# AcherStyx/SSD-Object-Detection

Hardware: AMD Instinct MI355X
Metric: images/sec SSD300 train step, batch 64 (higher is better)
Workload: dtype bf16; 1 GPU; BASELINE configs[2]: SSD300 full train step (anchor match+encode, image normalisation, conv fwd, loss, conv bwd, per-variable clip (64 variables) + Adam), per-GPU batch 64, 80 classes, synthetic COCO-shaped boxes; per_gpu_batch=64, global_batch=64, parallelism=single

## Files before the change

### ssd-object-detection_amd/csrc/conv.hip

```cpp
#include <atomic>
#include <climits>
#include <cstdint>
#include <cstring>
#include <type_traits>
#include "common.h"
#include <hip/hip_bf16.h>
#include <stdlib.h>

namespace {

}
#include "conv_common.h"
namespace {

template <int EPI>
__global__ void k_igemm_finalize(ConvGeom g, Epilogue ep) {
    const int n4 = (g.N + 3) >> 2;
    const long long idx = (long long)blockIdx.x * blockDim.x + threadIdx.x;
    if (idx >= (long long)g.M * n4) return;
    const int m = (int)(idx / n4), n = (int)(idx - (long long)m * n4) * 4;
    const bool full = n + 3 < g.N;
    float v[4] = {0.f, 0.f, 0.f, 0.f};
    if (full && !(g.N & 3)) {
        for (int z = 0; z < ep.ksplit; ++z) {
// ... 395 lines not shown
        for (int c = 0; c < 2; ++c) { fw1[c][0] = ldf(cb + OFF_W1 + wf0 + c * 2048); fw1[c][1] = ldf(cb + OFF_W1 + wf1 + c * 2048); }
        if constexpr (!(ABL & 1)) issue_w(cb + OFF_W0, 0);
        SSD_PHASE_MMA(0, 1, fw1)
#pragma unroll
        for (int p = 0; p < 4; ++p) { fx[p][0] = ldf(cb + OFF_X1 + xf0 + p * 2048); fx[p][1] = ldf(cb + OFF_X1 + xf1 + p * 2048); }
        if constexpr (!(ABL & 1)) issue_x(cb + OFF_X0, 0);
        SSD_PHASE_MMA(1, 1, fw1)
        if constexpr (!(ABL & 1)) issue_w(cb + OFF_W1, 1);
        wq += 8;
        asm volatile("s_waitcnt vmcnt(6)" ::: "memory");
        SSD_PHASE_MMA(1, 0, fw0)
    }
#undef SSD_PHASE_MMA
    if (wr == 0) __builtin_amdgcn_s_barrier();

    if (staged_ok<EPI>(g, ep) && !(g.ablate & 8)) {
        asm volatile("s_waitcnt vmcnt(0)" ::: "memory");
        auto row_to_m = [&](int row) { const int m = m0 + row; return m < g.M ? m : -1; };
        staged_epilogue<EPI, 256, 256, 4, 8, 512>(acc, smem, g, ep, n0, wr * 128, wc * 64, tid, row_to_m);
        return;
    }
    int mrow[8];
#pragma unroll
    for (int p = 0; p < 8; ++p) {
        const int m = m0 + wr * 128 + p * 16 + (lane & 15);
        mrow[p] = m < g.M ? m : -1;
    }
    conv_epilogue_rows<EPI, 4, 8>(acc, g, ep, mrow, n0 + wc * 64, lane);
}

constexpr int PATCH_W = 18;
constexpr int PATCH_PIX = PATCH_W * PATCH_W;

__device__ __forceinline__ bf16x8_t lds_read_b128_scoped(const char* __restrict__ p, const char* __restrict__ other) {
    (void)other;
    return *reinterpret_cast<const bf16x8_t*>(p);
}
constexpr int P32_PITCH = 96;
constexpr int P32_PATCH = 32 * 1024;

template <int BN, int EPI, bool FLAT>
__global__ __launch_bounds__(512) __attribute__((amdgpu_waves_per_eu(4, 4))) void k_conv3x3_patch32(
    const bf16_raw* __restrict__ x, const bf16_raw* __restrict__ w, ConvGeom g, Epilogue ep, int tiles_x, int tiles_y, int nblocks, int rowflat) {
    constexpr int CT = BN / 32;
    constexpr int PT = 4;
    constexpr int WBYTES = BN * 64;
    constexpr int OFF_W = 2 * P32_PATCH;
    constexpr int OFF_DUMMY = OFF_W + 2 * WBYTES;
    extern __shared__ __attribute__((aligned(16))) char smem[];

    const int tid = threadIdx.x, lane = tid & 63;
    const int wave = __builtin_amdgcn_readfirstlane(tid >> 6);
    const int wave_m = wave & 3, wave_n = wave >> 2;
    const int ntn = (g.N + BN - 1) / BN;
    const int kx = blockIdx.x >> 3;
    const int pblock = (kx / ntn) * 8 + (blockIdx.x & 7);
    if (pblock >= nblocks) return;
    const int n0 = (kx % ntn) * BN;
    constexpr bool flat = FLAT;
    const int Q = FLAT ? g.W + 2 : PATCH_W;
    const int img = (g.H + 1) * Q;
    int b = 0, y0 = 0, x0 = 0, f0 = 0;
    if constexpr (FLAT) {
        f0 = pblock * 256;
    } else {
        int t = pblock;
        const int tx = t % tiles_x; t /= tiles_x;
        x0 = tx * 16;
        if (rowflat) { y0 = t * 16; }
        else { const int ty = t % tiles_y; b = t / tiles_y; y0 = ty * 16; }
    }
    auto image_row = [&](int r) {
        if (!rowflat) { const int y = y0 + r; return (unsigned)y < (unsigned)g.H ? b * g.H + y : -1; }
        const int R = y0 + r;
        if (R < 0) return -1;
        const int bb = fdiv(R, g.d_h1), yy = R - bb * (g.H + 1);
        return (bb < g.B && yy < g.H) ? bb * g.H + yy : -1;
    };
    auto flat_pixel = [&](int f) {
        if (f < 0) return -1;
        const int bb = f / img;
        const int r = f - bb * img;
        const int yy = r / Q, xx = r - yy * Q - 1;
        return (bb < g.B && yy < g.H && (unsigned)xx < (unsigned)g.W) ? (bb * g.H + yy) * g.W + xx : -1;
    };

    const __amdgpu_buffer_rsrc_t xres = __builtin_amdgcn_make_buffer_rsrc((void*)x, 0, (unsigned)g.B * g.H * g.W * g.C * 2u, 0x00020000);
    const __amdgpu_buffer_rsrc_t wres = __builtin_amdgcn_make_buffer_rsrc((void*)w, 0, (unsigned)g.N * (unsigned)g.ldw * 2u, 0x00020000);
    constexpr unsigned OOB = 0xfffffff0u;
    unsigned pvo[4];
#pragma unroll
    for (int j = 0; j < 4; ++j) {
        const int q = (wave + 8 * j) * 64 + lane;
        const int pp = q / 6, sl = q - pp * 6;
        int pix;
        if (flat) {
            pix = pp < 256 + 2 * (Q + 1) ? flat_pixel(f0 - (Q + 1) + pp) : -1;
        } else {
            const int py = pp / PATCH_W, px = pp - py * PATCH_W;
            const int ix = x0 - 1 + px;
            const int ir = pp < PATCH_PIX ? image_row(py - 1) : -1;
            pix = (ir >= 0 && (unsigned)ix < (unsigned)g.W) ? ir * g.W + ix : -1;
        }
        pvo[j] = (sl < 4 && pix >= 0) ? ((unsigned)pix * (unsigned)g.C + (unsigned)(sl * 8)) * 2u : OOB;
    }
    unsigned wvo;
    {
        const int row = 16 * wave + (lane >> 2);
        const int piece = (lane & 3) ^ ((-(row >> 2)) & 3);
        const int n = n0 + (BN == 64 ? (row & 63) : row);
        wvo = (row < (BN == 64 ? 128 : BN) && n < g.N) ? ((unsigned)n * (unsigned)g.ldw + (unsigned)(piece * 8)) * 2u : OOB;
    }
    const int wdst = wave < BN / 16 ? wave * 1024 : -1;
    const int nchunk = g.C >> 5;

    unsigned pstash[3];
    pstash[0] = pvo[1]; pstash[1] = pvo[2]; pstash[2] = pvo[3];
    asm volatile("" ::"v"(&pstash[0]) : "memory");
    const unsigned pvo0 = pvo[0];
    auto dma_patch = [&](int chunk, int buf) {
        const unsigned o1 = pstash[0], o2 = pstash[1], o3 = pstash[2];
        char* dst = smem + buf * P32_PATCH + wave * 1024;
        __builtin_amdgcn_raw_ptr_buffer_load_lds(xres, (lds_void*)dst, 16, pvo0, chunk * 64, 0, 0);
        __builtin_amdgcn_raw_ptr_buffer_load_lds(xres, (lds_void*)(dst + 8 * 1024), 16, o1, chunk * 64, 0, 0);
        __builtin_amdgcn_raw_ptr_buffer_load_lds(xres, (lds_void*)(dst + 16 * 1024), 16, o2, chunk * 64, 0, 0);
        __builtin_amdgcn_raw_ptr_buffer_load_lds(xres, (lds_void*)(dst + 24 * 1024), 16, o3, chunk * 64, 0, 0);
    };
    auto dma_w = [&](int chunk, int tap, int buf) {
        char* dst = wdst >= 0 ? smem + OFF_W + buf * WBYTES + wdst : smem + OFF_DUMMY;
        __builtin_amdgcn_raw_ptr_buffer_load_lds(wres, (lds_void*)dst, 16, wvo, (tap * g.C + chunk * 32) * 2, 0, 0);
    };

    f32x4_t acc[CT][PT];
#pragma unroll
    for (int c = 0; c < CT; ++c)
#pragma unroll
        for (int p = 0; p < PT; ++p) acc[c][p] = f32x4_t{0.f, 0.f, 0.f, 0.f};

    const int frow = lane & 15, fk = lane >> 4;
    const int xbase = (flat ? 4 * wave_m * 16 + frow : 4 * wave_m * PATCH_W + frow) * P32_PITCH + fk * 16;
    constexpr int prow = (FLAT ? 16 : PATCH_W) * P32_PITCH;
    int wbase;
    {
        const int row = wave_n * (16 * CT) + frow;
        wbase = OFF_W + row * 64 + ((fk ^ ((-(row >> 2)) & 3)) << 4);
    }
    auto ldf = [&](int addr) { return *reinterpret_cast<const bf16x8_t*>(smem + addr); };

    if constexpr (BN == 64) {
        constexpr int WB2 = 2 * WBYTES;
        auto dma_w2 = [&](int chunk, int step, int buf) {
            const int tap = 2 * step + (wave >> 2);
            __builtin_amdgcn_raw_ptr_buffer_load_lds(wres, (lds_void*)(smem + OFF_W + buf * WB2 + wave * 1024), 16,
                                                     tap <= 8 ? wvo : OOB, ((tap <= 8 ? tap : 8) * g.C + chunk * 32) * 2, 0, 0);
        };
        dma_patch(0, 0);
        dma_w2(0, 0, 0);
        for (int chunk = 0; chunk < nchunk; ++chunk) {
            const int pb = (chunk & 1) * P32_PATCH;
            const bool next_chunk = chunk + 1 < nchunk;
#pragma unroll
            for (int st = 0; st < 5; ++st) {
                const int sidx = chunk * 5 + st;
                const int wb = (sidx & 1) * WB2;
                if (st == 1 && next_chunk) asm volatile("s_waitcnt vmcnt(4) lgkmcnt(0)" ::: "memory");
                else asm volatile("s_waitcnt vmcnt(0) lgkmcnt(0)" ::: "memory");
                __builtin_amdgcn_s_barrier();
                if (!(g.ablate & 16)) {
                    if (st < 4) dma_w2(chunk, st + 1, (sidx + 1) & 1);
                    else if (next_chunk) dma_w2(chunk + 1, 0, (sidx + 1) & 1);
                }
                if (st == 0 && next_chunk && !(g.ablate & 32)) dma_patch(chunk + 1, (chunk + 1) & 1);
                bf16x8_t fx[2][PT], fw[2][CT];
#pragma unroll
                for (int t = 0; t < 2; ++t) {
                    const int tap = 2 * st + t;
                    if (tap > 8) continue;
                    const int tapoff = pb + xbase + ((tap / 3) * Q + tap % 3) * P32_PITCH;
#pragma unroll
                    for (int p = 0; p < PT; ++p) fx[t][p] = ldf(tapoff + p * prow);
#pragma unroll
                    for (int c = 0; c < CT; ++c) fw[t][c] = ldf(wb + wbase + t * WBYTES + c * 1024);
                }
                __builtin_amdgcn_s_setprio(0);
#pragma unroll
                for (int t = 0; t < 2; ++t) {
                    if (2 * st + t > 8) continue;
#pragma unroll
                    for (int c = 0; c < CT; ++c)
#pragma unroll
                        for (int p = 0; p < PT; ++p)
                            acc[c][p] = __builtin_amdgcn_mfma_f32_16x16x32_bf16(fw[t][c], fx[t][p], acc[c][p], 0, 0, 0);
                }
                __builtin_amdgcn_s_setprio(3);
            }
        }
    } else {
    dma_patch(0, 0);
    dma_w(0, 0, 0);
    for (int chunk = 0; chunk < nchunk; ++chunk) {
        const int pb = (chunk & 1) * P32_PATCH;
        const bool next_chunk = chunk + 1 < nchunk;
#pragma unroll
        for (int tap = 0; tap < 9; ++tap) {
            const int wb = ((chunk + tap) & 1) * WBYTES;
            if (tap == 1 && next_chunk) asm volatile("s_waitcnt vmcnt(4) lgkmcnt(0)" ::: "memory");
            else asm volatile("s_waitcnt vmcnt(0) lgkmcnt(0)" ::: "memory");
            __builtin_amdgcn_s_barrier();
            if (!(g.ablate & 16)) {
                if (tap < 8) dma_w(chunk, tap + 1, ((chunk + tap + 1) & 1));
                else if (next_chunk) dma_w(chunk + 1, 0, ((chunk + tap + 1) & 1));
            }
            if (tap == 0 && next_chunk && !(g.ablate & 32)) dma_patch(chunk + 1, (chunk + 1) & 1);
            bf16x8_t fx[PT], fw[CT];
            const int tapoff = pb + xbase + ((tap / 3) * Q + tap % 3) * P32_PITCH;
#pragma unroll
            for (int p = 0; p < PT; ++p) fx[p] = ldf(tapoff + p * prow);
#pragma unroll
            for (int c = 0; c < CT; ++c) fw[c] = ldf(wb + wbase + c * 1024);
            __builtin_amdgcn_s_setprio(0);
#pragma unroll
            for (int c = 0; c < CT; ++c)
#pragma unroll
                for (int p = 0; p < PT; ++p)
                    acc[c][p] = __builtin_amdgcn_mfma_f32_16x16x32_bf16(fw[c], fx[p], acc[c][p], 0, 0, 0);
            __builtin_amdgcn_s_setprio(3);
        }
    }
    }
    if (staged_ok<EPI>(g, ep) && !(g.ablate & 8)) {
        auto row_to_m = [&](int row) {
            if (flat) return flat_pixel(f0 + row);
            const int ir = image_row(row >> 4), xx = x0 + (row & 15);
            return (ir >= 0 && xx < g.Wo) ? ir * g.Wo + xx : -1;
        };
        auto pool_index = [&](int py, int px) -> long long {
            if (flat || rowflat) return -1;
            const int gy = (y0 >> 1) + py, gx = (x0 >> 1) + px;
            return (gy < ep.pool_h && gx < ep.pool_w) ? ((long long)b * ep.pool_h + gy) * ep.pool_w + gx : -1;
        };
        staged_epilogue<EPI, 256, BN, CT, PT, 512>(acc, smem, g, ep, n0, wave_m * 64, wave_n * (16 * CT), tid, row_to_m, pool_index);
        return;
    }
    int mrow[PT];
#pragma unroll
    for (int p = 0; p < PT; ++p) {
        if (flat) {
            mrow[p] = flat_pixel(f0 + (4 * wave_m + p) * 16 + (lane & 15));
        } else {
            const int ir = image_row(4 * wave_m + p), xx = x0 + (lane & 15);
            mrow[p] = (ir >= 0 && xx < g.Wo) ? ir * g.Wo + xx : -1;
        }
    }
    conv_epilogue_rows<EPI, CT, PT>(acc, g, ep, mrow, n0 + wave_n * (16 * CT), lane);
}

constexpr int P5_PIX = 34 * PATCH_W;
constexpr int P5_NDMA = (P5_PIX * 6 + 63) / 64;
constexpr int P5_PATCH = P5_NDMA * 1024;
constexpr int P5_WSLOT = 128 * 64;
constexpr int P5_OFF_W = 2 * P5_PATCH;
constexpr int P5_OFF_DUMMY = P5_OFF_W + 4 * P5_WSLOT;
constexpr int P5_LDS = P5_OFF_DUMMY + 1024;

template <int EPI, bool FLAT>
__global__ __launch_bounds__(512) void k_conv3x3_p512(const bf16_raw* __restrict__ x, const bf16_raw* __restrict__ w, ConvGeom g,
                                                      Epilogue ep, int tiles_x, int tiles_y, int nblocks, int rowflat) {
    constexpr int BN = 128, CT = 4, PT = 8;
    extern __shared__ __attribute__((aligned(16))) char smem[];
    const int tid = threadIdx.x, lane = tid & 63;
    const int wave = __builtin_amdgcn_readfirstlane(tid >> 6);
    const int wave_m = wave & 3, wave_n = wave >> 2;
    const int ntn = (g.N + BN - 1) / BN;
    const int kx = blockIdx.x >> 3;
    const int pblock = (kx / ntn) * 8 + (blockIdx.x & 7);
    if (pblock >= nblocks) return;
    const int n0 = (kx % ntn) * BN;
    const int Q = FLAT ? g.W + 2 : PATCH_W;
    const int img = (g.H + 1) * Q;
    int b = 0, y0 = 0, x0 = 0, f0 = 0;
    if constexpr (FLAT) {
        f0 = pblock * 512;
    } else {
        int t = pblock;
        const int tx = t % tiles_x; t /= tiles_x;
        x0 = tx * 16;
        if (rowflat) { y0 = t * 32; }
        else { const int ty = t % tiles_y; b = t / tiles_y; y0 = ty * 32; }
    }
    auto image_row = [&](int r) {
        if (!rowflat) { const int y = y0 + r; return (unsigned)y < (unsigned)g.H ? b * g.H + y : -1; }
        const int R = y0 + r;
        if (R < 0) return -1;
        const int bb = fdiv(R, g.d_h1), yy = R - bb * (g.H + 1);
        return (bb < g.B && yy < g.H) ? bb * g.H + yy : -1;
    };
    auto flat_pixel = [&](int f) {
        if (f < 0) return -1;
        const int bb = f / img;
        const int r = f - bb * img;
        const int yy = r / Q, xx = r - yy * Q - 1;
        return (bb < g.B && yy < g.H && (unsigned)xx < (unsigned)g.W) ? (bb * g.H + yy) * g.W + xx : -1;
    };
    const __amdgpu_buffer_rsrc_t xres = __builtin_amdgcn_make_buffer_rsrc((void*)x, 0, (unsigned)g.B * g.H * g.W * g.C * 2u, 0x00020000);
    const __amdgpu_buffer_rsrc_t wres = __builtin_amdgcn_make_buffer_rsrc((void*)w, 0, (unsigned)g.N * (unsigned)g.ldw * 2u, 0x00020000);
    constexpr unsigned OOB = 0xfffffff0u;
    unsigned pvo[8];
#pragma unroll
    for (int j = 0; j < 8; ++j) {
        const int q = (wave + 8 * j) * 64 + lane;
        const int pp = q / 6, sl = q - pp * 6;
        int pix;
        if constexpr (FLAT) {
            pix = pp < 512 + 2 * (Q + 1) ? flat_pixel(f0 - (Q + 1) + pp) : -1;
        } else {
            const int py = pp / PATCH_W, px = pp - py * PATCH_W;
            const int ix = x0 - 1 + px;
            const int ir = pp < P5_PIX ? image_row(py - 1) : -1;
            pix = (ir >= 0 && (unsigned)ix < (unsigned)g.W) ? ir * g.W + ix : -1;
        }
        pvo[j] = (sl < 4 && pix >= 0 && wave + 8 * j < P5_NDMA) ? ((unsigned)pix * (unsigned)g.C + (unsigned)(sl * 8)) * 2u : OOB;
    }
    unsigned wvo;
    {
        const int row = 16 * wave + (lane >> 2);
        const int piece = (lane & 3) ^ ((-(row >> 2)) & 3);
        const int n = n0 + row;
        wvo = n < g.N ? ((unsigned)n * (unsigned)g.ldw + (unsigned)(piece * 8)) * 2u : OOB;
        if (g.ablate & 16) wvo = OOB;
    }
    const int nchunk = g.C >> 5;
    const int nstep = nchunk * 9;
    auto dma_piece = [&](int chunk, int buf, int j, bool live) {
        char* dst = wave + 8 * j < P5_NDMA ? smem + buf * P5_PATCH + (wave + 8 * j) * 1024 : smem + P5_OFF_DUMMY;
        __builtin_amdgcn_raw_ptr_buffer_load_lds(xres, (lds_void*)dst, 16, live ? pvo[j] : OOB, chunk * 64, 0, 0);
    };
    auto dma_w = [&](int step) {
        const int st = step < nstep ? step : nstep - 1;
        const int ch = st / 9, tp = st - ch * 9;
        __builtin_amdgcn_raw_ptr_buffer_load_lds(wres, (lds_void*)(smem + P5_OFF_W + (step & 3) * P5_WSLOT + wave * 1024), 16, wvo,
                                                 (tp * g.C + ch * 32) * 2, 0, 0);
    };
    f32x4_t acc[CT][PT];
#pragma unroll
    for (int c = 0; c < CT; ++c)
#pragma unroll
        for (int p = 0; p < PT; ++p) acc[c][p] = f32x4_t{0.f, 0.f, 0.f, 0.f};

    const int frow = lane & 15, fk = lane >> 4;
    const int xbase = (FLAT ? 8 * wave_m * 16 + frow : 8 * wave_m * PATCH_W + frow) * P32_PITCH + fk * 16;
    constexpr int prow = (FLAT ? 16 : PATCH_W) * P32_PITCH;
    int wbase;
    {
        const int row = wave_n * 64 + frow;
        wbase = P5_OFF_W + row * 64 + ((fk ^ ((-(row >> 2)) & 3)) << 4);
    }
    auto ldf = [&](int addr) { return lds_read_b128_scoped(smem + addr, smem); };
    auto load_x = [&](bf16x8_t (&fx)[PT], int pb, int tap) {
        const int tapoff = pb + xbase + ((tap / 3) * Q + tap % 3) * P32_PITCH;
#pragma unroll
        for (int p = 0; p < PT; ++p) fx[p] = ldf(tapoff + p * prow);
    };
    auto load_w = [&](bf16x8_t (&fw)[CT], int step) {
        const int wb = (step & 3) * P5_WSLOT;
#pragma unroll
        for (int c = 0; c < CT; ++c) fw[c] = ldf(wb + wbase + c * 1024);
    };
#pragma unroll
    for (int j = 0; j < 8; ++j) dma_piece(0, 0, j, true);
    dma_w(0); dma_w(1); dma_w(2);
    bf16x8_t fxa[PT], fxb[PT], fwa[CT], fwb[CT];
    asm volatile("s_waitcnt vmcnt(2)" ::: "memory");
    __builtin_amdgcn_s_barrier();
    load_x(fxa, 0, 0);
    load_w(fwa, 0);
    auto run_chunk = [&](int chunk, auto par_tag) {
        constexpr int PAR = decltype(par_tag)::value;
        const int pb = (chunk & 1) * P5_PATCH;
        const bool next_chunk = chunk + 1 < nchunk && !(g.ablate & 32);
#pragma unroll
        for (int tap = 0; tap < 9; ++tap) {
            constexpr int NT[9] = {1, 3, 5, 5, 5, 3, 1, 1, 1};
            if (NT[tap] == 1) asm volatile("s_waitcnt vmcnt(1) lgkmcnt(0)" ::: "memory");
            else if (NT[tap] == 3) asm volatile("s_waitcnt vmcnt(3) lgkmcnt(0)" ::: "memory");
            else asm volatile("s_waitcnt vmcnt(5) lgkmcnt(0)" ::: "memory");
            __builtin_amdgcn_s_barrier();
            const int step = chunk * 9 + tap;
            dma_w(step + 3);
            if (tap < 4) {
                dma_piece(chunk + 1, (chunk + 1) & 1, 2 * tap, next_chunk);
                dma_piece(chunk + 1, (chunk + 1) & 1, 2 * tap + 1, next_chunk);
            }
            bf16x8_t (&fxc)[PT] = ((tap + PAR) & 1) ? fxb : fxa;
            bf16x8_t (&fxn)[PT] = ((tap + PAR) & 1) ? fxa : fxb;
            bf16x8_t (&fwc)[CT] = ((tap + PAR) & 1) ? fwb : fwa;
            bf16x8_t (&fwn)[CT] = ((tap + PAR) & 1) ? fwa : fwb;
            if (tap < 8) load_x(fxn, pb, tap + 1);
            else load_x(fxn, next_chunk ? (P5_PATCH - pb) : pb, next_chunk ? 0 : 8);
            load_w(fwn, step + 1 < nstep ? step + 1 : step);
#pragma unroll
            for (int c = 0; c < CT; ++c)
#pragma unroll
                for (int p = 0; p < PT; ++p)
                    acc[c][p] = __builtin_amdgcn_mfma_f32_16x16x32_bf16(fwc[c], fxc[p], acc[c][p], 0, 0, 0);
#define SSD_P5_GROUP(NM_) __builtin_amdgcn_sched_group_barrier(0x008, NM_, 0); __builtin_amdgcn_sched_group_barrier(0x100, 1, 0)
            SSD_P5_GROUP(2); SSD_P5_GROUP(2); SSD_P5_GROUP(2); SSD_P5_GROUP(2); SSD_P5_GROUP(2); SSD_P5_GROUP(2);
            SSD_P5_GROUP(2); SSD_P5_GROUP(2); SSD_P5_GROUP(2); SSD_P5_GROUP(2); SSD_P5_GROUP(2); SSD_P5_GROUP(2);
            __builtin_amdgcn_sched_group_barrier(0x008, 8, 0);
#undef SSD_P5_GROUP
            __builtin_amdgcn_sched_barrier(0);
        }
    };
    for (int chunk = 0; chunk < nchunk; chunk += 2) {
        run_chunk(chunk, std::integral_constant<int, 0>{});
        run_chunk(chunk + 1, std::integral_constant<int, 1>{});
    }
    asm volatile("s_waitcnt vmcnt(0) lgkmcnt(0)" ::: "memory");
    if (staged_ok<EPI>(g, ep)) {
        auto row_to_m = [&](int row) {
            if constexpr (FLAT) return flat_pixel(f0 + row);
            const int ir = image_row(row >> 4), xx = x0 + (row & 15);
            return (ir >= 0 && xx < g.Wo) ? ir * g.Wo + xx : -1;
        };
        auto pool_index = [&](int py, int px) -> long long {
            if (FLAT || rowflat) return -1;
            const int gy = (y0 >> 1) + py, gx = (x0 >> 1) + px;
            return (gy < ep.pool_h && gx < ep.pool_w) ? ((long long)b * ep.pool_h + gy) * ep.pool_w + gx : -1;
        };
        staged_epilogue<EPI, 512, BN, CT, PT, 512>(acc, smem, g, ep, n0, wave_m * 128, wave_n * 64, tid, row_to_m, pool_index);
        return;
    }
    int mrow[PT];
#pragma unroll
    for (int p = 0; p < PT; ++p) {
        if constexpr (FLAT) {
            mrow[p] = flat_pixel(f0 + (8 * wave_m + p) * 16 + (lane & 15));
        } else {
            const int ir = image_row(8 * wave_m + p), xx = x0 + (lane & 15);
            mrow[p] = (ir >= 0 && xx < g.Wo) ? ir * g.Wo + xx : -1;
        }
    }
    conv_epilogue_rows<EPI, CT, PT>(acc, g, ep, mrow, n0 + wave_n * 64, lane);
}

constexpr int C64_PITCH = 160;

constexpr int C64B_ROWS = 8;
constexpr int C64B_PATCH_PIX = (C64B_ROWS + 2) * PATCH_W;
constexpr int C64B_NDMA = (C64B_PATCH_PIX * 10 + 63) / 64;
constexpr int C64B_PATCH = C64B_NDMA * 1024;
constexpr int C64B_STAGE = 2 * C64B_PATCH;
constexpr int C64B_FRAG_DEPTH = 3;
constexpr int C64B_BIAS = C64B_STAGE + 128 * 128;
constexpr int C64B_LDS = C64B_BIAS + 256;

struct C64W0 {
    const bf16_raw* img;
    float* slab_w;
    float* slab_b;
};
constexpr int C64B_IMG = 6 * 256;
constexpr int C64B_W0_IMG = 2 * C64B_PATCH;
constexpr int C64B_W0_SUMS = C64B_W0_IMG + 2 * C64B_IMG;
constexpr int C64B_W0_LDS = C64B_W0_SUMS + 4 * 3 * 64 * 16;

typedef __attribute__((address_space(3))) s16x4_t lds_s16x4;
__device__ __forceinline__ s16x4_t lds_read_tr16_scoped(const char* __restrict__ p, const char* __restrict__ other) {
    (void)other;
    return __builtin_amdgcn_ds_read_tr16_b64_v4i16((lds_s16x4*)p);
}

template <int EPI, bool W0 = false>
__global__ __launch_bounds__(256) __attribute__((amdgpu_waves_per_eu(2, 2)))
void k_conv3x3_c64b(const bf16_raw* __restrict__ x, const bf16_raw* __restrict__ w, ConvGeom g, Epilogue ep, int tiles_x, int tiles_y,
                    C64W0 w0) {
    static_assert(!W0 || EPI == EPI_DGRAD, "the fused first-layer weight gradient belongs to the data gradient");
    extern __shared__ __attribute__((aligned(16))) char smem[];
    const int tid = threadIdx.x, lane = tid & 63;
    const int wave = __builtin_amdgcn_readfirstlane(tid >> 6);
    const int wave_m = wave & 1, wave_n = wave >> 1;
    const int nblocks = g.B * tiles_x * tiles_y;
    const __amdgpu_buffer_rsrc_t xres = __builtin_amdgcn_make_buffer_rsrc((void*)x, 0, (unsigned)g.B * g.H * g.W * 64u * 2u, 0x00020000);
    constexpr unsigned OOB = 0xfffffff0u;
    constexpr int NJ = (C64B_NDMA + 3) / 4;
    const __amdgpu_buffer_rsrc_t ires = __builtin_amdgcn_make_buffer_rsrc((void*)(W0 ? w0.img : x), 0, (unsigned)g.B * g.H * g.W * 16u, 0x00020000);

    int pcode[NJ];
#pragma unroll
    for (int j = 0; j < NJ; ++j) {
        const int q = (wave + 4 * j) * 64 + lane;
        const int pp = q / 10, sl = q - pp * 10;
        const int py = pp / PATCH_W, px = pp - py * PATCH_W;
        pcode[j] = (sl < 8 && pp < C64B_PATCH_PIX && wave + 4 * j < C64B_NDMA) ? ((py << 16) | (px << 8) | (sl * 16)) : -1;
    }
    auto issue_patch = [&](int t, int buf) {
        int r = t;
        const int tx = r % tiles_x; r /= tiles_x;
        const int ty = r % tiles_y;
        const int b = r / tiles_y;
#pragma unroll
        for (int j = 0; j < NJ; ++j) {
            if (wave + 4 * j < C64B_NDMA) {
                const int iy = ty * C64B_ROWS - 1 + (pcode[j] >> 16), ix = tx * 16 - 1 + ((pcode[j] >> 8) & 255);
                const bool ok = pcode[j] >= 0 && (unsigned)iy < (unsigned)g.H && (unsigned)ix < (unsigned)g.W;
                const unsigned off = (unsigned)((b * g.H + iy) * g.W + ix) * 128u + (unsigned)(pcode[j] & 255);
                __builtin_amdgcn_raw_ptr_buffer_load_lds(xres, (lds_void*)(smem + buf * C64B_PATCH + (wave + 4 * j) * 1024), 16,
                                                         ok ? off : OOB, 0, 0, 0);
            }
        }
        if constexpr (W0) {
#pragma unroll
            for (int j = 0; j < 2; ++j) {
                if (wave + 4 * j < 6) {
                    const int q = (wave + 4 * j) * 64 + lane, pp = q >> 1;
                    const int py = pp / PATCH_W, px = pp - py * PATCH_W;
                    const int iy = ty * C64B_ROWS - 1 + py, ix = tx * 16 - 1 + px;
                    const bool ok = pp < C64B_PATCH_PIX && (unsigned)iy < (unsigned)g.H && (unsigned)ix < (unsigned)g.W;
                    const unsigned off = (unsigned)((b * g.H + iy) * g.W + ix) * 16u + (unsigned)(q & 1) * 4u;
                    __builtin_amdgcn_raw_ptr_buffer_load_lds(ires, (lds_void*)(smem + C64B_W0_IMG + buf * C64B_IMG + (wave + 4 * j) * 256), 4,
                                                             ok ? off : OOB, 0, 0, 0);
                }
            }
        }
    };
    const bool xcd_order = (gridDim.x & 7) == 0 && !(g.ablate & 64);
    const int per_xcd = (nblocks + 7) >> 3, slots = gridDim.x >> 3;
    auto block_of = [&](int i) {
        if (!xcd_order) { const int t = blockIdx.x + i * gridDim.x; return t < nblocks ? t : -1; }
        const int lin = i * slots + ((int)blockIdx.x >> 3);
        const int t = ((int)blockIdx.x & 7) * per_xcd + lin;
        return (lin < per_xcd && t < nblocks) ? t : -1;
    };
    if (block_of(0) >= 0) issue_patch(block_of(0), 0);

    const int frow = lane & 15, fk = lane >> 4;
    bf16x8_t fw[2][9][2];
#pragma unroll
    for (int c = 0; c < 2; ++c) {
        const int n = wave_n * 32 + c * 16 + frow;
#pragma unroll
        for (int tap = 0; tap < 9; ++tap)
#pragma unroll
            for (int ks = 0; ks < 2; ++ks) {
                uint4 v = make_uint4(0, 0, 0, 0);
                if (n < g.N) v = *reinterpret_cast<const uint4*>(w + (unsigned)n * 576u + (unsigned)(tap * 64 + ks * 32 + fk * 8));
                fw[c][tap][ks] = *reinterpret_cast<const bf16x8_t*>(&v);
            }
    }
    const int xbase = (4 * wave_m * PATCH_W + frow) * C64_PITCH + fk * 16;
    if constexpr (EPI == EPI_FWD) {
        if (tid < 64) reinterpret_cast<float*>(smem + C64B_BIAS)[tid] = (ep.bias && tid < g.N) ? ep.bias[tid] : 0.f;
    }
    if constexpr (W0) {
        f32x4_t* sums = reinterpret_cast<f32x4_t*>(smem + C64B_W0_SUMS) + wave * 3 * 64 + lane;
#pragma unroll
        for (int nt = 0; nt < 3; ++nt) sums[nt * 64] = f32x4_t{0.f, 0.f, 0.f, 0.f};
    }

    unsigned mkn[4] = {0u, 0u, 0u, 0u};
    auto load_masks = [&](int t) {
        int r = t;
        const int tx = r % tiles_x; r /= tiles_x;
        const int ty = r % tiles_y;
        const int b = r / tiles_y;
#pragma unroll
        for (int p = 0; p < 4; ++p) {
            const int y = ty * C64B_ROWS + 4 * wave_m + p, xx = tx * 16 + (lane & 15);
            mkn[p] = 0u;
            if (y < g.Ho && xx < g.Wo)
                mkn[p] = *reinterpret_cast<const unsigned*>(ep.mask_bits + (long long)((b * g.Ho + y) * g.Wo + xx) * 8 + wave_n * 4);
        }
    };
    if constexpr (W0) { if (block_of(0) >= 0) load_masks(block_of(0)); }

    int it = 0, prev_st = 0;
    for (int t = block_of(0); t >= 0; t = block_of(++it)) {
        const int cur = it & 1;
        if (g.ablate & 2) {}
        else if (prev_st >= 6) asm volatile("s_waitcnt vmcnt(6) lgkmcnt(0)" ::: "memory");
        else if (prev_st == 5) asm volatile("s_waitcnt vmcnt(5) lgkmcnt(0)" ::: "memory");
        else if (prev_st == 4) asm volatile("s_waitcnt vmcnt(4) lgkmcnt(0)" ::: "memory");
        else if (prev_st == 3) asm volatile("s_waitcnt vmcnt(3) lgkmcnt(0)" ::: "memory");
        else if (prev_st == 2) asm volatile("s_waitcnt vmcnt(2) lgkmcnt(0)" ::: "memory");
        else if (prev_st == 1) asm volatile("s_waitcnt vmcnt(1) lgkmcnt(0)" ::: "memory");
        else asm volatile("s_waitcnt vmcnt(0) lgkmcnt(0)" ::: "memory");
        __syncthreads();
        __builtin_amdgcn_s_setprio(0);
        int r = t;
        const int tx = r % tiles_x; r /= tiles_x;
        const int ty = r % tiles_y;
        const int b = r / tiles_y;
        const int y0 = ty * C64B_ROWS, x0 = tx * 16;
        unsigned mk[4];
        auto chunk_pixel = [&](int t, int i) {
            const int y = y0 + 2 * i + (t >> 7), xx = x0 + ((t >> 3) & 15);
            return (y < g.Ho && xx < g.Wo) ? (b * g.Ho + y) * g.Wo + xx : -1;
        };
        const bool premask = EPI == EPI_DGRAD && ep.mask_bits != nullptr && !(g.ablate & 128);
        if constexpr (W0) {
#pragma unroll
            for (int p = 0; p < 4; ++p) mk[p] = mkn[p];
        } else if constexpr (EPI == EPI_DGRAD) {
#pragma unroll
            for (int i = 0; i < 4; ++i) {
                const int m = chunk_pixel(tid, i);
                mk[i] = 0u;
                if (premask && m >= 0) mk[i] = ep.mask_bits[(long long)m * 8 + (tid & 7)];
            }
        }
        const int tnext = block_of(it + 1);
        if (tnext >= 0 && !(g.ablate & 1)) issue_patch(tnext, cur ^ 1);
        if constexpr (W0) { if (tnext >= 0) load_masks(tnext); }
        const int pb = cur * C64B_PATCH + xbase;
        f32x4_t acc[2][4];
#pragma unroll
        for (int c = 0; c < 2; ++c) {
            f32x4_t a0 = f32x4_t{0.f, 0.f, 0.f, 0.f};
            if constexpr (EPI == EPI_FWD)
                a0 = *reinterpret_cast<const f32x4_t*>(smem + C64B_BIAS + (wave_n * 32 + c * 16 + (lane >> 4) * 4) * 4);
#pragma unroll
            for (int p = 0; p < 4; ++p) acc[c][p] = a0;
        }
        auto frag = [&](int s2) {
            return *reinterpret_cast<const bf16x8_t*>(smem + pb + ((s2 / 6) * PATCH_W + (s2 / 2) % 3) * C64_PITCH + (s2 & 1) * 64);
        };
        constexpr int FD = C64B_FRAG_DEPTH;
        bf16x8_t fr[FD];
#pragma unroll
        for (int i = 0; i < FD - 1; ++i) fr[i] = frag(i);
#pragma unroll
        for (int s2 = 0; s2 < 36; ++s2) {
            if (s2 + FD - 1 < 36) fr[(s2 + FD - 1) % FD] = frag(s2 + FD - 1);
            const int rr = s2 / 6, dx = (s2 / 2) % 3, ks = s2 & 1;
#pragma unroll
            for (int dy = 0; dy < 3; ++dy) {
                const int p = rr - dy;
                if (p >= 0 && p < 4) {
#pragma unroll
                    for (int c = 0; c < 2; ++c)
                        acc[c][p] = __builtin_amdgcn_mfma_f32_16x16x32_bf16(fw[c][dy * 3 + dx][ks], fr[s2 % FD], acc[c][p], 0, 0, 0);
                }
            }
            __builtin_amdgcn_sched_barrier(0);
        }
        __builtin_amdgcn_s_setprio(3);
        if (g.ablate & 8) {
#pragma unroll
            for (int c = 0; c < 2; ++c)
#pragma unroll
                for (int p = 0; p < 4; ++p) asm volatile("" :: "v"(acc[c][p]));
            prev_st = 0;
            continue;
        }
        auto row_to_m = [&](int row) {
            const int y = y0 + (row >> 4), xx = x0 + (row & 15);
            return (y < g.Ho && xx < g.Wo) ? (b * g.Ho + y) * g.Wo + xx : -1;
        };
        auto pool_index = [&](int py, int px) -> long long {
            const int gy = (y0 >> 1) + py, gx = (x0 >> 1) + px;
            return (gy < ep.pool_h && gx < ep.pool_w) ? ((long long)b * ep.pool_h + gy) * ep.pool_w + gx : -1;
        };
        if constexpr (W0) {
            char* st = smem + cur * C64B_PATCH;
            asm volatile("s_waitcnt lgkmcnt(0)" ::: "memory");
            __builtin_amdgcn_s_barrier();
            int t2 = tid;
            asm volatile("" : "+v"(t2));
            {
                const int l3 = t2 & 63;
#pragma unroll
                for (int c = 0; c < 2; ++c) {
                    const int col = wave_n * 32 + c * 16 + (l3 >> 4) * 4;
                    const int sh = 8 * (2 * c + (l3 >> 5)) + 4 * ((l3 >> 4) & 1);
#pragma unroll
                    for (int p = 0; p < 4; ++p) {
                        const int row = wave_m * 64 + p * 16 + (l3 & 15);
                        const unsigned bits = mk[p] >> sh;
                        const unsigned k0 = keep_mask2(bits, 0), k1 = keep_mask2(bits, 2);
                        lds_st8_scoped(st + row * 128 + ((((col >> 3) ^ row) & 7) << 4) + (col & 4) * 2, smem,
                            make_uint2((pack_bf16x2(acc[c][p][0], acc[c][p][1])) & k0,
                                       (pack_bf16x2(acc[c][p][2], acc[c][p][3])) & k1));
                    }
                }
            }
            asm volatile("s_waitcnt lgkmcnt(0)" ::: "memory");
            __builtin_amdgcn_s_barrier();
            int l2 = t2 & 63;
            const int gq = l2 >> 4, q = (l2 >> 2) & 3, p4 = l2 & 3;
            int db[2], ib[3];
#pragma unroll
            for (int h = 0; h < 2; ++h) {
                const int r = 8 * gq + q + 4 * h;
                db[h] = r * 128 + ((((2 * wave + (p4 >> 1)) ^ r) & 7) << 4) + (p4 & 1) * 8;
            }
#pragma unroll
            for (int nt = 0; nt < 3; ++nt) {
                int tap = 4 * nt + p4;
                if (tap > 8) tap = 8;
                ib[nt] = (((gq >> 1) + tap / 3) * PATCH_W + 8 * (gq & 1) + q + tap % 3) * 8;
            }
            const char* im = smem + C64B_W0_IMG + cur * C64B_IMG;
            f32x4_t* sums = reinterpret_cast<f32x4_t*>(smem + C64B_W0_SUMS) + wave * 3 * 64 + l2;
            f32x4_t aw[3];
#pragma unroll
            for (int nt = 0; nt < 3; ++nt) {
                const uint4 u = lds_ld16_scoped(reinterpret_cast<const char*>(sums + nt * 64), smem);
                aw[nt] = f32x4_t{__uint_as_float(u.x), __uint_as_float(u.y), __uint_as_float(u.z), __uint_as_float(u.w)};
            }
            bf16x8_t ones;
#pragma unroll
            for (int e = 0; e < 8; ++e) ones[e] = (__bf16)1.0f;
#pragma unroll
            for (int s = 0; s < 4; ++s) {
                bf16x8_t fd;
                reinterpret_cast<s16x4_t*>(&fd)[0] = lds_read_tr16_scoped(st + db[0] + s * 4096, smem);
                reinterpret_cast<s16x4_t*>(&fd)[1] = lds_read_tr16_scoped(st + db[1] + s * 4096, smem);
#pragma unroll
                for (int nt = 0; nt < 3; ++nt) {
                    bf16x8_t fp;
// ... 2106 lines not shown
```

Measured before the change: 7107 images/sec.

## Halve barriers in implicit-GEMM conv main loop by pairing taps per sync

Restructures the 3x3 conv main loop into 18-step periods, where each barrier covers two MFMA tap steps and a fixed schedule of weight and patch DMAs instead of one barrier per tap. Out-of-range patch loads are now disabled by building a zero-size buffer resource rather than substituting an out-of-bounds offset. The goal is to cut per-tap s_waitcnt/barrier overhead and keep the MFMA pipes busier. In exchange, the weight slots get less slack in the prefetch distance, and the period loop assumes nstep is a multiple of 18 (even chunk count), as the old loop did.

```diff
diff --git a/ssd-object-detection_amd/csrc/conv.hip b/ssd-object-detection_amd/csrc/conv.hip
--- a/ssd-object-detection_amd/csrc/conv.hip
+++ b/ssd-object-detection_amd/csrc/conv.hip
@@ -721,7 +721,7 @@
         const int yy = r / Q, xx = r - yy * Q - 1;
         return (bb < g.B && yy < g.H && (unsigned)xx < (unsigned)g.W) ? (bb * g.H + yy) * g.W + xx : -1;
     };
-    const __amdgpu_buffer_rsrc_t xres = __builtin_amdgcn_make_buffer_rsrc((void*)x, 0, (unsigned)g.B * g.H * g.W * g.C * 2u, 0x00020000);
+    const unsigned xbytes = (unsigned)g.B * g.H * g.W * g.C * 2u;
     const __amdgpu_buffer_rsrc_t wres = __builtin_amdgcn_make_buffer_rsrc((void*)w, 0, (unsigned)g.N * (unsigned)g.ldw * 2u, 0x00020000);
     constexpr unsigned OOB = 0xfffffff0u;
     unsigned pvo[8];
@@ -752,7 +752,8 @@
     const int nstep = nchunk * 9;
     auto dma_piece = [&](int chunk, int buf, int j, bool live) {
         char* dst = wave + 8 * j < P5_NDMA ? smem + buf * P5_PATCH + (wave + 8 * j) * 1024 : smem + P5_OFF_DUMMY;
-        __builtin_amdgcn_raw_ptr_buffer_load_lds(xres, (lds_void*)dst, 16, live ? pvo[j] : OOB, chunk * 64, 0, 0);
+        const __amdgpu_buffer_rsrc_t res = __builtin_amdgcn_make_buffer_rsrc((void*)x, 0, live ? xbytes : 0u, 0x00020000);
+        __builtin_amdgcn_raw_ptr_buffer_load_lds(res, (lds_void*)dst, 16, pvo[j], chunk * 64, 0, 0);
     };
     auto dma_w = [&](int step) {
         const int st = step < nstep ? step : nstep - 1;
@@ -793,47 +794,55 @@
     __builtin_amdgcn_s_barrier();
     load_x(fxa, 0, 0);
     load_w(fwa, 0);
-    auto run_chunk = [&](int chunk, auto par_tag) {
-        constexpr int PAR = decltype(par_tag)::value;
-        const int pb = (chunk & 1) * P5_PATCH;
-        const bool next_chunk = chunk + 1 < nchunk && !(g.ablate & 32);
-#pragma unroll
-        for (int tap = 0; tap < 9; ++tap) {
-            constexpr int NT[9] = {1, 3, 5, 5, 5, 3, 1, 1, 1};
-            if (NT[tap] == 1) asm volatile("s_waitcnt vmcnt(1) lgkmcnt(0)" ::: "memory");
-            else if (NT[tap] == 3) asm volatile("s_waitcnt vmcnt(3) lgkmcnt(0)" ::: "memory");
-            else asm volatile("s_waitcnt vmcnt(5) lgkmcnt(0)" ::: "memory");
+    auto run_period = [&](int s0) {
+        const int c0 = s0 / 9;
+        const bool live2 = c0 + 2 < nchunk;
+#pragma unroll
+        for (int j = 0; j < 9; ++j) {
+            constexpr int PV[9] = {3, 3, 2, 0, 3, 3, 2, 0, 0};
+            const int NV = PV[(j + 8) % 9];
+            if (NV == 0) asm volatile("s_waitcnt vmcnt(0) lgkmcnt(0)" ::: "memory");
+            else if (NV == 2) asm volatile("s_waitcnt vmcnt(2) lgkmcnt(0)" ::: "memory");
+            else asm volatile("s_waitcnt vmcnt(3) lgkmcnt(0)" ::: "memory");
             __builtin_amdgcn_s_barrier();
-            const int step = chunk * 9 + tap;
-            dma_w(step + 3);
-            if (tap < 4) {
-                dma_piece(chunk + 1, (chunk + 1) & 1, 2 * tap, next_chunk);
-                dma_piece(chunk + 1, (chunk + 1) & 1, 2 * tap + 1, next_chunk);
-            }
-            bf16x8_t (&fxc)[PT] = ((tap + PAR) & 1) ? fxb : fxa;
-            bf16x8_t (&fxn)[PT] = ((tap + PAR) & 1) ? fxa : fxb;
-            bf16x8_t (&fwc)[CT] = ((tap + PAR) & 1) ? fwb : fwa;
-            bf16x8_t (&fwn)[CT] = ((tap + PAR) & 1) ? fwa : fwb;
-            if (tap < 8) load_x(fxn, pb, tap + 1);
-            else load_x(fxn, next_chunk ? (P5_PATCH - pb) : pb, next_chunk ? 0 : 8);
-            load_w(fwn, step + 1 < nstep ? step + 1 : step);
+            const int s = s0 + 2 * j;
+            dma_w(s + 3);
+            dma_w(s + 4);
+            if (PV[j]) {
+                const int pc = j < 4 ? c0 + 1 : c0 + 2;
+                const bool live = (j < 4 || live2) && !(g.ablate & 32);
+                const int p0 = (j & 3) * 3;
+#pragma unroll
+                for (int i = 0; i < PV[j]; ++i) dma_piece(pc, pc & 1, p0 + i, live);
+            }
+            const int l1 = 2 * j + 1, l2 = 2 * j + 2;
+            load_x(fxb, l1 >= 9 ? P5_PATCH : 0, l1 % 9);
+            load_w(fwb, s + 1);
 #pragma unroll
             for (int c = 0; c < CT; ++c)
 #pragma unroll
                 for (int p = 0; p < PT; ++p)
-                    acc[c][p] = __builtin_amdgcn_mfma_f32_16x16x32_bf16(fwc[c], fxc[p], acc[c][p], 0, 0, 0);
+                    acc[c][p] = __builtin_amdgcn_mfma_f32_16x16x32_bf16(fwa[c], fxa[p], acc[c][p], 0, 0, 0);
 #define SSD_P5_GROUP(NM_) __builtin_amdgcn_sched_group_barrier(0x008, NM_, 0); __builtin_amdgcn_sched_group_barrier(0x100, 1, 0)
-            SSD_P5_GROUP(2); SSD_P5_GROUP(2); SSD_P5_GROUP(2); SSD_P5_GROUP(2); SSD_P5_GROUP(2); SSD_P5_GROUP(2);
-            SSD_P5_GROUP(2); SSD_P5_GROUP(2); SSD_P5_GROUP(2); SSD_P5_GROUP(2); SSD_P5_GROUP(2); SSD_P5_GROUP(2);
-            __builtin_amdgcn_sched_group_barrier(0x008, 8, 0);
+#define SSD_P5_STEP_ORDER()                                                                                              \
+            SSD_P5_GROUP(2); SSD_P5_GROUP(2); SSD_P5_GROUP(2); SSD_P5_GROUP(2); SSD_P5_GROUP(2); SSD_P5_GROUP(2);      \
+            SSD_P5_GROUP(2); SSD_P5_GROUP(2); SSD_P5_GROUP(2); SSD_P5_GROUP(2); SSD_P5_GROUP(2); SSD_P5_GROUP(2);      \
+            __builtin_amdgcn_sched_group_barrier(0x008, 8, 0);    \
+            __builtin_amdgcn_sched_barrier(0)
+            SSD_P5_STEP_ORDER();
+            load_x(fxa, l2 >= 18 ? 0 : (l2 >= 9 ? P5_PATCH : 0), l2 % 9);
+            load_w(fwa, s + 2);
+#pragma unroll
+            for (int c = 0; c < CT; ++c)
+#pragma unroll
+                for (int p = 0; p < PT; ++p)
+                    acc[c][p] = __builtin_amdgcn_mfma_f32_16x16x32_bf16(fwb[c], fxb[p], acc[c][p], 0, 0, 0);
+            SSD_P5_STEP_ORDER();
+#undef SSD_P5_STEP_ORDER
 #undef SSD_P5_GROUP
-            __builtin_amdgcn_sched_barrier(0);
         }
     };
-    for (int chunk = 0; chunk < nchunk; chunk += 2) {
-        run_chunk(chunk, std::integral_constant<int, 0>{});
-        run_chunk(chunk + 1, std::integral_constant<int, 1>{});
-    }
+    for (int s0 = 0; s0 < nstep; s0 += 18) run_period(s0);
     asm volatile("s_waitcnt vmcnt(0) lgkmcnt(0)" ::: "memory");
     if (staged_ok<EPI>(g, ep)) {
         auto row_to_m = [&](int row) {
```

After: 7132 images/sec (median of 6 runs). No clear change (+0.3%).
